# chzchzchz/raftsql

Measured on NVIDIA B200. Metric: raft_ticks_per_sec_1Mx5, higher is better.
Workload: dtype u64

## Files before the change

raftsql_b200/csrc/mrq_kernels.cuh:

```cuda
#pragma once

#include <cuda_runtime.h>
#include <stdint.h>

#include "../../include/mrq.h"
#include "../../include/mrq_packed8.h"
#include "../../include/mrq_trace.h"

namespace mrq {

static constexpr uint64_t kNoGate = 0xFFFFFFFFFFFFFFFFull;

struct Meta {
  uint32_t role, lead, vote, self, elapsed, rto, hb, votes, strict, ltok;
};
__host__ __device__ __forceinline__ uint64_t meta_pack(const Meta &m) {
  return (uint64_t)(m.role & 3u) | ((uint64_t)(m.lead & 15u) << 2) | ((uint64_t)(m.vote & 15u) << 6) |
         ((uint64_t)(m.self & 15u) << 10) | ((uint64_t)(m.elapsed & 0xFFFu) << 14) |
         ((uint64_t)(m.rto & 0xFFFu) << 26) | ((uint64_t)(m.hb & 0xFFu) << 38) |
         ((uint64_t)(m.votes & 0xFFFFu) << 46) | ((uint64_t)(m.strict & 1u) << 62) | ((uint64_t)(m.ltok & 1u) << 63);
}
__host__ __device__ __forceinline__ Meta meta_unpack(uint64_t w) {
  Meta m;
  m.role = (uint32_t)(w & 3u);
// ... 31 lines not shown
  uint64_t *tick_next;
  uint32_t election_tick, heartbeat_tick;
  uint8_t *peer_lo[8];
  uint64_t *peer_full[8];
  uint32_t world, rank, gather_prime;
  uint32_t l2_policy;
  uint32_t *slow_list;
  unsigned *slow_count, *slow_count_next;
};

__device__ __forceinline__ void pdl_launch_dependents() { asm volatile("griddepcontrol.launch_dependents;"); }
__device__ __forceinline__ void pdl_wait() { asm volatile("griddepcontrol.wait;" ::: "memory"); }

template <class Args>
__device__ __forceinline__ void gather_store(const Args &a, const uint64_t i, const uint64_t committed, const uint64_t committed0) {
  const uint64_t at = (uint64_t)a.rank * a.G + i;
  const bool full = a.gather_prime || ((committed ^ committed0) >> 8) != 0;
#pragma unroll 1
  for (uint32_t p = 0; p < a.world; ++p) {
    a.peer_lo[p][at] = (uint8_t)committed;
    if (full) a.peer_full[p][at] = committed;
  }
}

#ifndef MRQ_HOST_EMULATION
__device__ __forceinline__ uint64_t ld_stream(const uint64_t *p) {
  uint64_t v;
  asm volatile("ld.global.nc.L1::no_allocate.u64 %0, [%1];" : "=l"(v) : "l"(p));
  return v;
}
__device__ __forceinline__ uint32_t ld_stream_u8(const uint8_t *p) {
  uint32_t v;
  asm volatile("ld.global.nc.L1::no_allocate.u8 %0, [%1];" : "=r"(v) : "l"(p));
  return v;
}
__device__ __forceinline__ uint32_t ld_stream_u32(const uint32_t *p) {
  uint32_t v;
  asm volatile("ld.global.nc.L1::no_allocate.u32 %0, [%1];" : "=r"(v) : "l"(p));
  return v;
}
__device__ __forceinline__ uint64_t ld_state(const uint64_t *p) {
  uint64_t v;
  asm volatile("ld.global.L1::no_allocate.u64 %0, [%1];" : "=l"(v) : "l"(p));
  return v;
}
__device__ __forceinline__ void st_state(uint64_t *p, uint64_t v) {
  asm volatile("st.global.L1::no_allocate.u64 [%0], %1;" ::"l"(p), "l"(v) : "memory");
}
__device__ __forceinline__ void st_state_u32(uint32_t *p, uint32_t v) {
  asm volatile("st.global.L1::no_allocate.u32 [%0], %1;" ::"l"(p), "r"(v) : "memory");
}

__device__ __forceinline__ uint64_t l2_policy(uint32_t kind) {
  uint64_t p;
  if (kind == 1u)
    asm volatile("createpolicy.fractional.L2::evict_first.b64 %0, 1.0;" : "=l"(p));
  else if (kind == 2u)
    asm volatile("createpolicy.fractional.L2::evict_last.b64 %0, 1.0;" : "=l"(p));
  else
    asm volatile("createpolicy.fractional.L2::evict_normal.b64 %0, 1.0;" : "=l"(p));
  return p;
}
__device__ __forceinline__ uint64_t ld_stream_p(const uint64_t *p, uint64_t pol) {
  uint64_t v;
  asm volatile("ld.global.nc.L1::no_allocate.L2::cache_hint.u64 %0, [%1], %2;" : "=l"(v) : "l"(p), "l"(pol));
  return v;
}
__device__ __forceinline__ uint32_t ld_stream_u8_p(const uint8_t *p, uint64_t pol) {
  uint32_t v;
  asm volatile("ld.global.nc.L1::no_allocate.L2::cache_hint.u8 %0, [%1], %2;" : "=r"(v) : "l"(p), "l"(pol));
  return v;
}
__device__ __forceinline__ uint32_t ld_stream_u32_p(const uint32_t *p, uint64_t pol) {
  uint32_t v;
  asm volatile("ld.global.nc.L1::no_allocate.L2::cache_hint.u32 %0, [%1], %2;" : "=r"(v) : "l"(p), "l"(pol));
  return v;
}
__device__ __forceinline__ uint64_t ld_state_p(const uint64_t *p, uint64_t pol) {
  uint64_t v;
  asm volatile("ld.global.L1::no_allocate.L2::cache_hint.u64 %0, [%1], %2;" : "=l"(v) : "l"(p), "l"(pol));
  return v;
}
__device__ __forceinline__ void st_state_p(uint64_t *p, uint64_t v, uint64_t pol) {
  asm volatile("st.global.L1::no_allocate.L2::cache_hint.u64 [%0], %1, %2;" ::"l"(p), "l"(v), "l"(pol) : "memory");
}
__device__ __forceinline__ void st_state_u32_p(uint32_t *p, uint32_t v, uint64_t pol) {
  asm volatile("st.global.L1::no_allocate.L2::cache_hint.u32 [%0], %1, %2;" ::"l"(p), "r"(v), "l"(pol) : "memory");
}
#else
inline uint64_t ld_stream(const uint64_t *p) { return *p; }
inline uint32_t ld_stream_u8(const uint8_t *p) { return *p; }
inline uint32_t ld_stream_u32(const uint32_t *p) { return *p; }
inline uint64_t ld_state(const uint64_t *p) { return *p; }
inline void st_state(uint64_t *p, uint64_t v) { *p = v; }
inline void st_state_u32(uint32_t *p, uint32_t v) { *p = v; }
inline uint64_t l2_policy(uint32_t) { return 0; }
inline uint64_t ld_stream_p(const uint64_t *p, uint64_t) { return *p; }
inline uint32_t ld_stream_u8_p(const uint8_t *p, uint64_t) { return *p; }
inline uint32_t ld_stream_u32_p(const uint32_t *p, uint64_t) { return *p; }
inline uint64_t ld_state_p(const uint64_t *p, uint64_t) { return *p; }
inline void st_state_p(uint64_t *p, uint64_t v, uint64_t) { *p = v; }
inline void st_state_u32_p(uint32_t *p, uint32_t v, uint64_t) { *p = v; }
#endif

__device__ __forceinline__ void cswap_desc(uint64_t &hi, uint64_t &lo) {
  const uint64_t a = hi, b = lo;
  const bool sw = a < b;
  hi = sw ? b : a;
  lo = sw ? a : b;
}
template <int R>
__device__ __forceinline__ uint64_t quorum_index64(const uint64_t (&m)[R]) {
  constexpr int Q = R / 2 + 1;
  uint64_t v[R];
#pragma unroll
  for (int i = 0; i < R; ++i) v[i] = m[i];
#pragma unroll
  for (int p = 0; p < Q; ++p) {
#pragma unroll
    for (int i = R - 1; i > p; --i) cswap_desc(v[i - 1], v[i]);
  }
  return v[Q - 1];
}
template <int R>
__device__ __forceinline__ uint32_t quorum_index32(const uint32_t (&d)[R]) {
  constexpr int Q = R / 2 + 1;
  if constexpr (R == 1) {
    return d[0];
  } else if constexpr (R == 2) {
    return min(d[0], d[1]);
  } else if constexpr (R == 3) {
    return max(min(d[0], d[1]), min(max(d[0], d[1]), d[2]));
  } else if constexpr (R == 5) {
    const uint32_t lo_ab = min(d[0], d[1]), hi_ab = max(d[0], d[1]);
    const uint32_t lo_cd = min(d[2], d[3]), hi_cd = max(d[2], d[3]);
    const uint32_t f = max(lo_ab, lo_cd), g = min(hi_ab, hi_cd);
    return max(min(d[4], f), min(max(d[4], f), g));
  } else {
    uint32_t v[R];
#pragma unroll
    for (int i = 0; i < R; ++i) v[i] = d[i];
#pragma unroll
    for (int p = 0; p < Q; ++p) {
#pragma unroll
      for (int i = R - 1; i > p; --i) {
        const uint32_t a = v[i - 1], b = v[i];
        v[i - 1] = max(a, b);
        v[i] = min(a, b);
      }
    }
    return v[Q - 1];
  }
}
__device__ __forceinline__ void delta32(uint64_t m, uint64_t c, uint32_t &d, uint32_t &bad) {
  uint32_t lo, hi, b;
#ifndef MRQ_HOST_EMULATION
  asm("sub.cc.u32 %0, %3, %5;\n\t"
      "subc.cc.u32 %1, %4, %6;\n\t"
      "subc.u32 %2, 0, 0;"
      : "=r"(lo), "=r"(hi), "=r"(b)
      : "r"((uint32_t)m), "r"((uint32_t)(m >> 32)), "r"((uint32_t)c), "r"((uint32_t)(c >> 32)));
#else
  const uint64_t diff = m - c;
  lo = (uint32_t)diff;
  hi = (uint32_t)(diff >> 32);
  b = m < c ? 0xFFFFFFFFu : 0u;
#endif
  d = ((b | hi) == 0u) ? lo : 0u;
  bad |= ~b & hi;
}
template <int R>
__device__ __forceinline__ uint64_t quorum_index(const uint64_t (&m)[R], uint64_t committed) {
  uint32_t d[R];
  uint32_t bad = 0;
#pragma unroll
  for (int r = 0; r < R; ++r) delta32(m[r], committed, d[r], bad);
  if (__builtin_expect(bad == 0u, 1)) return committed + quorum_index32<R>(d);
  return quorum_index64<R>(m);
}

enum : uint32_t {
  D_TERM = 1u << 0, D_LI = 1u << 1, D_LT = 1u << 2, D_COMMIT = 1u << 3, D_GATE = 1u << 4, D_MATCH0 = 1u << 8
};

template <int R>
struct Group {
  uint64_t term, last_index, last_term, committed, gate;
  uint64_t match[R];
  uint32_t role, lead, vote, self, elapsed, rto, hb, votes, strict, ltok;
  uint32_t out, dirty, ev;
  bool lt_valid;
  bool pending;
  const uint64_t *lt_ptr;
  uint64_t seed, gg, tick_no;
  uint32_t et, ht;

  static constexpr uint32_t Q = R / 2 + 1;
  enum : uint32_t { EV_CAMPAIGN = 1, EV_WON = 2, EV_STEPDOWN = 4, EV_COMMIT = 8, EV_GRANT = 16, EV_ERROR = 32 };

  __device__ __forceinline__ uint64_t lastTerm() {
    if (!lt_valid) {
      last_term = ltok ? term : ld_state(lt_ptr);
      lt_valid = true;
    }
    return last_term;
  }
  __device__ __forceinline__ void setSelfMatch(uint64_t v) {
#pragma unroll
    for (int r = 0; r < R; ++r)
      if ((uint32_t)(r + 1) == self && match[r] != v) {
        match[r] = v;
        dirty |= D_MATCH0 << r;
      }
  }
  __device__ __forceinline__ bool maybeCommit() {
    const uint64_t mci = quorum_index<R>(match, committed);
    if (mci > committed && mci >= gate && mci <= last_index) {
      committed = mci;
      dirty |= D_COMMIT;
      out |= MRQ_OUT_COMMIT_ADVANCED;
      ev |= EV_COMMIT;
      return true;
    }
    return false;
  }
  __device__ __forceinline__ void flushCommit() {
    if (pending) {
      pending = false;
      if (maybeCommit()) out |= MRQ_OUT_BCAST_APPEND;
    }
  }
  __device__ __forceinline__ void reset(uint64_t t) {
    if (term != t) {
      term = t;
      vote = 0;
      ltok = 0;
      dirty |= D_TERM;
    }
    lead = 0;
    elapsed = 0;
    hb = 0;
    votes = 0;
    rto = mrq_randomized_timeout(seed, gg, tick_no, et);
  }
  __device__ __forceinline__ void becomeFollower(uint64_t t, uint32_t ld) {
    flushCommit();
    if (role != MRQ_ROLE_FOLLOWER) {
      out |= MRQ_OUT_STEPPED_DOWN;
      ev |= EV_STEPDOWN;
    }
    reset(t);
    lead = ld;
    role = MRQ_ROLE_FOLLOWER;
    if (gate != kNoGate) {
      gate = kNoGate;
      dirty |= D_GATE;
    }
  }
  __device__ __forceinline__ void appendEntry(uint32_t n) {
    last_index += n;
    dirty |= D_LI;
    if (!ltok && (!lt_valid || last_term != term)) {
      last_term = term;
      lt_valid = true;
      dirty |= D_LT;
    }
    ltok = 1;
    setSelfMatch(last_index);
    pending = false;
    maybeCommit();
  }
  __device__ __forceinline__ void becomeLeader() {
    reset(term);
    lead = self;
    role = MRQ_ROLE_LEADER;
    strict = 0;
    pending = false;
    out |= MRQ_OUT_BECAME_LEADER;
    ev |= EV_WON;
#pragma unroll
    for (int r = 0; r < R; ++r) {
      match[r] = 0;
      dirty |= D_MATCH0 << r;
    }
    gate = last_index + 1;
    dirty |= D_GATE;
    appendEntry(1);
  }
  __device__ __forceinline__ void campaign() {
    reset(term + 1);
    vote = self;
    role = MRQ_ROLE_CANDIDATE;
    ev |= EV_CAMPAIGN;
    votes |= 1u << (2u * (self - 1u));
    if (Q == 1u) {
      becomeLeader();
      return;
    }
    out |= MRQ_OUT_CAMPAIGN;
  }
  __device__ __forceinline__ void commitTo(uint64_t c) {
    if (committed < c) {
      if (last_index < c) {
        ev |= EV_ERROR;
        return;
      }
// ... 571 lines not shown
  for (unsigned it = 0; it < rounds; ++it, k += stride) {
    uint32_t ev = 0;
    if (k < n) ev = general_group_tick<R>(a, (uint64_t)a.slow_list[k]);
    if (__any_sync(0xFFFFFFFFu, ev != 0)) count_events(a.ctr, ev);
  }
}

struct Tick8Args {
  TickArgs t;
  Inbox8 b;
};
template <int R>
__global__ void __launch_bounds__(kTickThreads, (R <= 5 ? 8 : (R == 6 ? 7 : 6))) tick_fast8_kernel(const Tick8Args a8) {
  const TickArgs &a = a8.t;
  pdl_launch_dependents();
  const uint64_t i = (uint64_t)blockIdx.x * blockDim.x + threadIdx.x;
  uint32_t ev = 0;
  bool slow = false;
  pdl_wait();
  if (blockIdx.x == 0 && threadIdx.x == 0) *a.tick_next = *a.tick_cur + 1;
  fast_group_tick8<R>(a, a8.b, i, slow, ev);
  const unsigned smask = __ballot_sync(0xFFFFFFFFu, slow);
  if (smask != 0) {
    const unsigned lane = threadIdx.x & 31u;
    unsigned base = 0;
    if (lane == 0) base = atomicAdd(a.slow_count, (unsigned)__popc(smask));
    base = __shfl_sync(0xFFFFFFFFu, base, 0);
    if (slow) a.slow_list[base + __popc(smask & ((1u << lane) - 1u))] = (uint32_t)i;
  }
  if (__any_sync(0xFFFFFFFFu, ev != 0)) count_events(a.ctr, ev);
}
template <int R>
__global__ void __launch_bounds__(kTickThreads, (R <= 5 ? 6 : 5)) tick_slow8_kernel(const Tick8Args a8) {
  const TickArgs &a = a8.t;
  pdl_launch_dependents();
  pdl_wait();
  const unsigned n = *a.slow_count;
  if (blockIdx.x == 0 && threadIdx.x == 0) *a.slow_count_next = 0;
  const unsigned stride = gridDim.x * blockDim.x;
  const unsigned rounds = (n + stride - 1) / stride;
  unsigned k = blockIdx.x * blockDim.x + threadIdx.x;
  for (unsigned it = 0; it < rounds; ++it, k += stride) {
    uint32_t ev = 0;
    if (k < n) ev = general_group_tick8<R>(a, a8.b, (uint64_t)a.slow_list[k]);
    if (__any_sync(0xFFFFFFFFu, ev != 0)) count_events(a.ctr, ev);
  }
}

template <int R>
__global__ void __launch_bounds__(kTickThreads, (R <= 5 ? 6 : 5)) tick_fused_kernel(const TickArgs a) {
  __shared__ uint32_t s_list[kTickThreads];
  __shared__ unsigned s_n;
  pdl_launch_dependents();
  const uint64_t base = (uint64_t)blockIdx.x * blockDim.x;
  uint32_t ev = 0;
  bool slow = false;
  if (threadIdx.x == 0) s_n = 0;
  pdl_wait();
  if (blockIdx.x == 0 && threadIdx.x == 0) *a.tick_next = *a.tick_cur + 1;
  fast_group_tick<R>(a, base + threadIdx.x, slow, ev);
  __syncthreads();
  const unsigned smask = __ballot_sync(0xFFFFFFFFu, slow);
  if (smask != 0) {
    const unsigned lane = threadIdx.x & 31u;
    unsigned pos = 0;
    if (lane == 0) pos = atomicAdd(&s_n, (unsigned)__popc(smask));
    pos = __shfl_sync(0xFFFFFFFFu, pos, 0);
    if (slow) s_list[pos + __popc(smask & ((1u << lane) - 1u))] = threadIdx.x;
  }
  __syncthreads();
  const unsigned n = s_n;
  if (__any_sync(0xFFFFFFFFu, ev != 0)) count_events(a.ctr, ev);
  if (n != 0) {
    uint32_t ev2 = 0;
    if (threadIdx.x < n) ev2 = general_group_tick<R>(a, base + s_list[threadIdx.x]);
    if (__any_sync(0xFFFFFFFFu, ev2 != 0)) count_events(a.ctr, ev2);
  }
}

template <int R>
__global__ void __launch_bounds__(kTickThreads, (R <= 5 ? 6 : 5)) tick_general_kernel(const TickArgs a) {
  pdl_launch_dependents();
  const uint64_t i = (uint64_t)blockIdx.x * blockDim.x + threadIdx.x;
  pdl_wait();
  if (blockIdx.x == 0 && threadIdx.x == 0) *a.tick_next = *a.tick_cur + 1;
  uint32_t ev = 0;
  if (i < a.G) ev = general_group_tick<R>(a, i);
  if (__any_sync(0xFFFFFFFFu, ev != 0)) count_events(a.ctr, ev);
}

enum : uint32_t { CF_COMPACT = 1u, CF_TERM_OK = 2u, CF_GATE_OPEN = 4u };
enum : uint32_t { CD_META = 1u, CD_COMMIT = 2u, CD_WIN = 4u, CD_MATCH0 = 1u << 8, CD_MATCH_ANY = 0xFFu << 8 };
#ifndef MRQ_HOST_EMULATION
static constexpr uint32_t kCompactSpan = 0x7FFFFFFFu;
#else
static uint32_t kCompactSpan = 0x7FFFFFFFu;
#endif

struct CompactView {
  uint8_t *flag;
  uint32_t *commit;
  uint32_t *win;
  uint32_t *gate;
  uint32_t *iblo;
  uint32_t *match;
  uint64_t *ibase;
};

template <int R>
struct CGroup {
  uint64_t meta;
  uint32_t commit, win;
  uint32_t m[R];
};

__host__ __device__ __forceinline__ uint32_t crow_sender(uint32_t j, uint32_t self_id) {
  return j + (j + 1u >= self_id ? 1u : 0u);
}

template <int R>
__device__ __forceinline__ bool compact_hot_step(CGroup<R> &g, const uint32_t flag, const uint32_t (&wb)[R > 1 ? R - 1 : 1],
                                                 const uint32_t nprop, const uint32_t gate, const uint32_t et, const uint32_t ht,
                                                 uint32_t &out, uint32_t &adv, uint32_t &dirty) {
  constexpr uint64_t kSettled = 3ull | (1ull << 62) | (1ull << 63);
  bool hot = (flag & (CF_COMPACT | CF_TERM_OK)) == (CF_COMPACT | CF_TERM_OK) &&
             (g.meta & kSettled) == ((uint64_t)MRQ_ROLE_LEADER | (1ull << 63));
  uint32_t li = g.m[R - 1];
  hot = hot && li + nprop <= kCompactSpan;
  uint32_t nm[R];
  uint32_t d = 0, min_ack = MRQ_P8_NO_ACK, kinds = 0, mx_max = 0, moved = 0;
#pragma unroll
  for (int j = 0; j < R - 1; ++j) {
    const uint32_t w = wb[j];
    kinds |= w;
    const bool ack = (w & 1u) != 0u;
    const uint32_t pay = w >> 2;
    const uint32_t mx = ack ? g.win + pay : 0u;
    mx_max = max(mx_max, mx);
    nm[j] = max(g.m[j], mx);
    moved |= nm[j] ^ g.m[j];
    min_ack = ack ? min(min_ack, pay) : min_ack;
  }
  if (!hot || mx_max > li || (kinds & 2u) != 0u) return false;
  uint32_t o = 0;
  li += nprop;
  nm[R - 1] = li;
  if (nprop) {
    moved = 1u;
    o |= MRQ_OUT_BCAST_APPEND;
  }
  d = moved != 0u ? CD_MATCH0 : 0u;
  uint32_t commit = g.commit, q = 0;
  if (d != 0u) {
    uint32_t dl[R];
#pragma unroll
    for (int r = 0; r < R; ++r) dl[r] = max(nm[r], commit) - commit;
    q = quorum_index32<R>(dl);
    const bool open = (flag & CF_GATE_OPEN) != 0u || commit + q >= gate;
    q = (commit + q <= li && open) ? q : 0u;
  }
  if (q != 0u) {
    commit += q;
    d |= CD_COMMIT;
    o |= MRQ_OUT_COMMIT_ADVANCED | MRQ_OUT_BCAST_APPEND;
  }
  uint32_t lo = (uint32_t)g.meta, hi = (uint32_t)(g.meta >> 32);
  uint32_t el = ((lo >> 14) & 0xFFFu) + 1u;
  el = el >= et ? 0u : el;
  lo = (lo & ~(0xFFFu << 14)) | (el << 14);
  if (ht <= 1u) {
    hi &= ~(0xFFu << 6);
    o |= MRQ_OUT_BCAST_HEARTBEAT;
  } else {
    uint32_t hb = ((hi >> 6) & 0xFFu) + 1u;
    if (hb >= ht) {
      hb = 0;
      o |= MRQ_OUT_BCAST_HEARTBEAT;
    }
    hi = (hi & ~(0xFFu << 6)) | (hb << 6);
  }
  const uint64_t nmeta = ((uint64_t)hi << 32) | lo;
  d |= nmeta != g.meta ? CD_META : 0u;
  if (min_ack < MRQ_P8_NO_ACK && min_ack > MRQ_P8_SLACK) {
    g.win += min_ack - MRQ_P8_SLACK;
    d |= CD_WIN;
  }
  g.meta = nmeta;
  g.commit = commit;
#pragma unroll
  for (int r = 0; r < R; ++r) g.m[r] = nm[r];
  out = o;
  adv = q;
  dirty = d;
  return true;
}

template <int R>
__device__ __forceinline__ bool compact_step(CGroup<R> &g, const uint32_t flag, const uint32_t (&wb)[R > 1 ? R - 1 : 1],
                                             const uint32_t nprop, const uint32_t gate, const uint32_t et, const uint32_t ht,
                                             uint32_t &out, uint32_t &adv, uint32_t &dirty) {
  out = 0;
  adv = 0;
  dirty = 0;
  if (!(flag & CF_COMPACT)) return true;
  Meta m = meta_unpack(g.meta);
  uint32_t kind[R > 1 ? R - 1 : 1], pay[R > 1 ? R - 1 : 1];
  bool any_ack = false, any_hb = false;
  uint32_t min_ack = MRQ_P8_NO_ACK;
#pragma unroll
  for (int j = 0; j < R - 1; ++j) {
    kind[j] = wb[j] & 3u;
    pay[j] = (wb[j] >> 2) & 63u;
    if (kind[j] == 1u) {
      any_ack = true;
      min_ack = pay[j] < min_ack ? pay[j] : min_ack;
    } else if (kind[j] == 3u) {
      any_hb = true;
    } else if (kind[j] == 2u && (pay[j] <= 2u || pay[j] == 63u)) {
      return true;
    } else {
      kind[j] = 0;
    }
  }
  uint32_t li = g.m[R - 1];
  CGroup<R> n = g;
  if (m.role == MRQ_ROLE_LEADER) {
    if (m.strict || !m.ltok || any_hb) return true;
    if (any_ack && !(flag & CF_TERM_OK)) return true;
    if (li + nprop > kCompactSpan) return true;
    bool changed = false;
#pragma unroll
    for (int j = 0; j < R - 1; ++j)
      if (kind[j] == 1u) {
        const uint32_t mx = g.win + pay[j];
        if (mx > li) return true;
        if (n.m[j] < mx) {
          n.m[j] = mx;
          dirty |= CD_MATCH0 << j;
          changed = true;
        }
      }
    if (nprop) {
      li += nprop;
      n.m[R - 1] = li;
      dirty |= CD_MATCH0 << (R - 1);
      out |= MRQ_OUT_BCAST_APPEND;
      changed = true;
    }
    if (changed) {
      uint32_t d[R];
#pragma unroll
      for (int r = 0; r < R; ++r) d[r] = max(n.m[r], n.commit) - n.commit;
      const uint32_t q = quorum_index32<R>(d);
      const uint32_t mci = n.commit + q;
      if (q != 0u && mci <= li && ((flag & CF_GATE_OPEN) != 0u || mci >= gate)) {
        adv = q;
        n.commit = mci;
        dirty |= CD_COMMIT;
        out |= MRQ_OUT_COMMIT_ADVANCED | MRQ_OUT_BCAST_APPEND;
      }
    }
    ++m.hb;
    ++m.elapsed;
    if (m.elapsed >= et) m.elapsed = 0;
    if (m.hb >= ht) {
      m.hb = 0;
      out |= MRQ_OUT_BCAST_HEARTBEAT;
    }
  } else if (m.role == MRQ_ROLE_FOLLOWER) {
    if (nprop != 0u || any_ack) return true;
    if (any_hb && !(flag & CF_TERM_OK)) return true;
#pragma unroll
    for (int j = 0; j < R - 1; ++j)
      if (kind[j] == 3u && (crow_sender((uint32_t)j, m.self) + 1u != m.lead || g.win + pay[j] > li)) return true;
    if ((any_hb ? 1u : m.elapsed + 1u) >= m.rto) return true;
#pragma unroll
    for (int j = 0; j < R - 1; ++j)
      if (kind[j] == 3u) {
        const uint32_t mx = g.win + pay[j];
        if (n.commit < mx) {
          adv += mx - n.commit;
          n.commit = mx;
          dirty |= CD_COMMIT;
          out |= MRQ_OUT_COMMIT_ADVANCED;
        }
        out |= 1u << (MRQ_OUT_ACK_REPLY_SHIFT + crow_sender((uint32_t)j, m.self));
      }
    m.elapsed = any_hb ? 1u : m.elapsed + 1u;
  } else {
    return true;
  }
  if (min_ack < MRQ_P8_NO_ACK && min_ack > MRQ_P8_SLACK) {
    n.win = g.win + (min_ack - MRQ_P8_SLACK);
    dirty |= CD_WIN;
  }
  n.meta = meta_pack(m);
  if (n.meta != g.meta) dirty |= CD_META;
  g = n;
  return false;
}

__device__ __forceinline__ void materialise_group(const StateView &s, const CompactView &c, uint64_t *base_index, uint64_t gs, uint32_t R,
                                                  const uint64_t i) {
  if (!(c.flag[i] & CF_COMPACT)) return;
  const Meta m = meta_unpack(s.meta[i]);
  const uint64_t ib = c.ibase[i];
  s.committed[i] = ib + c.commit[i];
  base_index[i] = ib + c.win[i];
  s.last_index[i] = ib + c.match[(uint64_t)(R - 1u) * gs + i];
  if (m.role == MRQ_ROLE_LEADER) {
    s.match[(uint64_t)(m.self - 1u) * gs + i] = ib + c.match[(uint64_t)(R - 1u) * gs + i];
    for (uint32_t j = 0; j + 1u < R; ++j) {
      const uint32_t v = c.match[(uint64_t)j * gs + i];
      if (v != 0u) s.match[(uint64_t)crow_sender(j, m.self) * gs + i] = ib + v;
    }
  }
}

__device__ __forceinline__ void compact_group(const StateView &s, const CompactView &c, const uint64_t *base_index,
                                              const uint64_t *base_term, uint64_t gs, uint32_t R, const uint64_t i) {
  const Meta m = meta_unpack(s.meta[i]);
  const uint64_t li = s.last_index[i], cm = s.committed[i], wb = base_index[i], gate = s.term_start[i];
  const uint64_t lo = cm < wb ? cm : wb;
  const uint64_t ib = lo ? lo - 1u : 0u;
  bool fits = m.self >= 1 && m.self <= R && !m.strict && cm <= li && li - ib <= (uint64_t)kCompactSpan &&
              wb - ib <= (uint64_t)kCompactSpan;
  const bool leader = m.role == MRQ_ROLE_LEADER;
  if (fits && leader) fits = s.match[(uint64_t)(m.self - 1u) * gs + i] == li;
  if (!fits) {
    c.flag[i] = 0;
    return;
  }
  c.ibase[i] = ib;
  c.iblo[i] = (uint32_t)ib;
  c.commit[i] = (uint32_t)(cm - ib);
  c.win[i] = (uint32_t)(wb - ib);
  for (uint32_t j = 0; j + 1u < R; ++j) {
    uint32_t v = 0;
    if (leader) {
      const uint64_t mv = s.match[(uint64_t)crow_sender(j, m.self) * gs + i];
      v = mv > ib ? (uint32_t)(mv - ib) : 0u;
    }
    c.match[(uint64_t)j * gs + i] = v;
  }
  c.match[(uint64_t)(R - 1u) * gs + i] = (uint32_t)(li - ib);
  uint32_t go = 0xFFFFFFFFu;
  if (leader) go = gate > ib ? (gate - ib > 0xFFFFFFFEull ? 0xFFFFFFFFu : (uint32_t)(gate - ib)) : 0u;
  c.gate[i] = go;
  c.flag[i] = (uint8_t)(CF_COMPACT | (base_term[i] == s.term[i] ? CF_TERM_OK : 0u) | ((leader && gate <= cm) ? CF_GATE_OPEN : 0u));
}

struct TickDesc {
  const uint8_t *word8;
  const uint8_t *prop8;
  InboxView in;
  uint32_t *out;
  uint8_t *delta;
};
static constexpr uint32_t kMaxTicksPerLaunch = 96;
struct Tick4Args {
  TickArgs t;
  CompactView c;
  uint64_t *base_index;
  const uint64_t *base_term;
  TickDesc d0;
  const TickDesc *descs;
  uint32_t nticks;
  uint32_t write_through;
  unsigned long long *slow_list64;
};

template <int R>
__device__ __forceinline__ uint32_t slow_group_ticks_c(const Tick4Args &A, const uint64_t i, const uint32_t t0) {
  const TickArgs &a0 = A.t;
  materialise_group(a0.s, A.c, A.base_index, a0.gs, (uint32_t)R, i);
  uint32_t ev = 0;
  const uint64_t tick0 = *a0.tick_cur;
  for (uint32_t t = t0; t < A.nticks; ++t) {
    const TickDesc d = A.descs ? A.descs[t] : A.d0;
    TickArgs a = a0;
    a.in = d.in;
    a.s.out = d.out;
    const uint64_t c0 = a.s.committed[i];
    const Inbox8 b{d.word8, d.prop8, A.base_index, A.base_term};
    ev |= general_group_tick8<R>(a, b, i, tick0 + t);
    const uint64_t adv = a.s.committed[i] - c0;
    d.delta[i] = (uint8_t)(adv > 255u ? 255u : adv);
  }
  compact_group(a0.s, A.c, A.base_index, A.base_term, a0.gs, (uint32_t)R, i);
  return ev;
}

#ifndef MRQ_HOST_EMULATION
template <int R>
struct CStepResult {
  CGroup<R> g;
  uint32_t out, adv, dirty, slow;
};
template <int R>
__device__ __noinline__ CStepResult<R> compact_step_cold(CGroup<R> g, uint32_t flag, uint32_t w0123, uint32_t w4567, uint32_t nprop,
                                                         uint32_t gate, uint32_t et, uint32_t ht) {
  uint32_t wb[R > 1 ? R - 1 : 1];
#pragma unroll
  for (int j = 0; j < (R > 1 ? R - 1 : 1); ++j) wb[j] = ((j < 4 ? w0123 : w4567) >> (8 * (j & 3))) & 0xFFu;
  CStepResult<R> r;
  r.slow = compact_step<R>(g, flag, wb, nprop, gate, et, ht, r.out, r.adv, r.dirty) ? 1u : 0u;
  r.g = g;
  return r;
}
#endif

#ifndef MRQ_HOST_EMULATION
struct u32x4 {
  uint32_t v[4];
};
__device__ __forceinline__ u32x4 ld_v4u32_p(const uint32_t *p, uint64_t pol) {
  u32x4 r;
  asm volatile("ld.global.L1::no_allocate.L2::cache_hint.v4.u32 {%0, %1, %2, %3}, [%4], %5;"
               : "=r"(r.v[0]), "=r"(r.v[1]), "=r"(r.v[2]), "=r"(r.v[3])
               : "l"(p), "l"(pol));
  return r;
}
__device__ __forceinline__ void st_v4u32_p(uint32_t *p, const u32x4 &r, uint64_t pol) {
  asm volatile("st.global.L1::no_allocate.L2::cache_hint.v4.u32 [%0], {%1, %2, %3, %4}, %5;" ::"l"(p), "r"(r.v[0]), "r"(r.v[1]),
               "r"(r.v[2]), "r"(r.v[3]), "l"(pol)
               : "memory");
}
__device__ __forceinline__ void ld_v2u64_p(const uint64_t *p, uint64_t pol, uint64_t &a, uint64_t &b) {
  asm volatile("ld.global.L1::no_allocate.L2::cache_hint.v2.u64 {%0, %1}, [%2], %3;" : "=l"(a), "=l"(b) : "l"(p), "l"(pol));
}
__device__ __forceinline__ void st_v2u64_p(uint64_t *p, uint64_t a, uint64_t b, uint64_t pol) {
  asm volatile("st.global.L1::no_allocate.L2::cache_hint.v2.u64 [%0], {%1, %2}, %3;" ::"l"(p), "l"(a), "l"(b), "l"(pol) : "memory");
}

template <int R, int THREADS>
#ifndef MRQ_T4_THREADS_PER_SM
#define MRQ_T4_THREADS_PER_SM 512
#endif
__global__ void __launch_bounds__(THREADS, (R <= 5 ? MRQ_T4_THREADS_PER_SM : 384) / THREADS) tick_fast4_kernel(const Tick4Args A) {
  const TickArgs &a = A.t;
  pdl_launch_dependents();
  const uint64_t i0 = ((uint64_t)blockIdx.x * blockDim.x + threadIdx.x) * 4u;
  const bool active = i0 < a.gs;
  const uint64_t i = active ? i0 : 0;
  const uint64_t pol_stream = l2_policy(a.l2_policy ? 1u : 0u);
  const uint64_t pol_keep = l2_policy(a.l2_policy ? 2u : 0u);
  pdl_wait();
  if (blockIdx.x == 0 && threadIdx.x == 0) *a.tick_next = *a.tick_cur + A.nticks;
  CGroup<R> g[4];
  uint32_t flag[4];
  {
    const uint32_t fw = ld_stream_u32_p(reinterpret_cast<const uint32_t *>(A.c.flag + i), pol_keep);
    ld_v2u64_p(a.s.meta + i, pol_keep, g[0].meta, g[1].meta);
    ld_v2u64_p(a.s.meta + i + 2, pol_keep, g[2].meta, g[3].meta);
    const u32x4 cm = ld_v4u32_p(A.c.commit + i, pol_keep);
    const u32x4 wn = ld_v4u32_p(A.c.win + i, pol_keep);
    u32x4 mv[R];
#pragma unroll
    for (int r = 0; r < R; ++r) mv[r] = ld_v4u32_p(A.c.match + (uint64_t)r * a.gs + i, pol_keep);
#pragma unroll
    for (int k = 0; k < 4; ++k) {
      flag[k] = (fw >> (8 * k)) & 0xFFu;
      g[k].commit = cm.v[k];
      g[k].win = wn.v[k];
#pragma unroll
      for (int r = 0; r < R; ++r) g[k].m[r] = mv[r].v[k];
    }
  }
  uint32_t stopped = 0;
#pragma unroll
  for (int k = 0; k < 4; ++k)
    if (!active || i0 + k >= a.G) stopped |= 1u << k;
  u32x4 gate{};
  if (((flag[0] & flag[1] & flag[2] & flag[3]) & CF_GATE_OPEN) == 0u) gate = ld_v4u32_p(A.c.gate + i, pol_keep);
  const bool gather = a.world > 1;
  u32x4 iblo{};
  if (gather) iblo = ld_v4u32_p(A.c.iblo + i, pol_keep);
  uint32_t acc_dirty = 0, ncommit = 0;
  __shared__ TickDesc s_desc[kMaxTicksPerLaunch];
  if (A.descs) {
    const uint32_t nw = A.nticks * (uint32_t)(sizeof(TickDesc) / 4);
    for (uint32_t w = threadIdx.x; w < nw; w += THREADS) reinterpret_cast<uint32_t *>(s_desc)[w] = reinterpret_cast<const uint32_t *>(A.descs)[w];
  } else if (threadIdx.x == 0) {
    s_desc[0] = A.d0;
  }
  __syncthreads();
  constexpr int NW = R > 1 ? R - 1 : 1;
  auto load_frame = [&](uint32_t t, uint32_t (&w)[NW], uint32_t &pbytes) {
    const TickDesc &dd = s_desc[t];
#pragma unroll
    for (int j = 0; j < R - 1; ++j) w[j] = ld_stream_u32_p(reinterpret_cast<const uint32_t *>(dd.word8 + (uint64_t)j * a.gs + i), pol_stream);
    if (R == 1) w[0] = 0;
    pbytes = dd.prop8 ? ld_stream_u32_p(reinterpret_cast<const uint32_t *>(dd.prop8 + i), pol_stream) : 0u;
  };
  uint32_t wb[NW], pb, wb1[NW], pb1 = 0;
  load_frame(0, wb, pb);
#pragma unroll
  for (int j = 0; j < NW; ++j) wb1[j] = 0;
  if (A.nticks > 1) load_frame(1, wb1, pb1);
  for (uint32_t t = 0; t < A.nticks; ++t) {
    uint32_t wb2[NW], pb2 = 0;
#pragma unroll
    for (int j = 0; j < NW; ++j) wb2[j] = 0;
    if (t + 2 < A.nticks) load_frame(t + 2, wb2, pb2);
    const TickDesc &d = s_desc[t];
    u32x4 outw{};
    uint32_t dw = 0, newly = 0, tdirty = 0;
    u32x4 lo_old{};
    if (gather) {
#pragma unroll
      for (int k = 0; k < 4; ++k) lo_old.v[k] = iblo.v[k] + g[k].commit;
    }
#pragma unroll
    for (int k = 0; k < 4; ++k) {
      if (stopped & (1u << k)) continue;
      uint32_t wk[R > 1 ? R - 1 : 1];
#pragma unroll
      for (int j = 0; j < (R > 1 ? R - 1 : 1); ++j) wk[j] = (wb[j] >> (8 * k)) & 0xFFu;
      uint32_t o, adv, dirty;
      const uint32_t np = (pb >> (8 * k)) & 0xFFu;
      bool slow = false;
      if (!compact_hot_step<R>(g[k], flag[k], wk, np, gate.v[k], a.election_tick, a.heartbeat_tick, o, adv, dirty)) {
        uint32_t p0 = 0, p1 = 0;
#pragma unroll
        for (int j = 0; j < R - 1; ++j) {
          if (j < 4) p0 |= wk[j] << (8 * j);
          else p1 |= wk[j] << (8 * (j - 4));
        }
        const CStepResult<R> cr = compact_step_cold<R>(g[k], flag[k], p0, p1, np, gate.v[k], a.election_tick, a.heartbeat_tick);
        g[k] = cr.g;
        o = cr.out;
        adv = cr.adv;
        dirty = cr.dirty;
        slow = cr.slow != 0u;
      }
      if (slow) {
        newly |= 1u << k;
      } else {
        outw.v[k] = o;
        dw |= (adv > 255u ? 255u : adv) << (8 * k);
        tdirty |= dirty;
        ncommit += adv != 0u;
      }
    }
    if (__any_sync(0xFFFFFFFFu, newly != 0u)) {
#pragma unroll
      for (int k = 0; k < 4; ++k) {
        const bool s = (newly >> k) & 1u;
        const unsigned smask = __ballot_sync(0xFFFFFFFFu, s);
        if (smask != 0) {
          const unsigned lane = threadIdx.x & 31u;
          unsigned base = 0;
          if (lane == 0) base = atomicAdd(a.slow_count, (unsigned)__popc(smask));
          base = __shfl_sync(0xFFFFFFFFu, base, 0);
          if (s) A.slow_list64[base + __popc(smask & ((1u << lane) - 1u))] = ((unsigned long long)t << 32) | (unsigned long long)(i0 + k);
        }
      }
      stopped |= newly;
    }
    acc_dirty |= tdirty;
    if (active) {
      st_v4u32_p(d.out + i, outw, pol_stream);
      st_state_u32_p(reinterpret_cast<uint32_t *>(d.delta + i), dw, pol_stream);
      if (gather) {
        uint32_t lo4 = 0;
        bool carry = false;
        u32x4 lo;
#pragma unroll
        for (int k = 0; k < 4; ++k) {
          lo.v[k] = iblo.v[k] + g[k].commit;
          lo4 |= (lo.v[k] & 0xFFu) << (8 * k);
          carry = carry || ((lo.v[k] ^ lo_old.v[k]) >> 8) != 0u;
        }
        const uint64_t at = (uint64_t)a.rank * a.G + i;
        const bool whole = i0 + 3 < a.G && (at & 3u) == 0u && stopped == 0u;
#pragma unroll 1
        for (uint32_t p = 0; p < a.world; ++p) {
          if (whole) {
            st_state_u32_p(reinterpret_cast<uint32_t *>(a.peer_lo[p] + at), lo4, pol_stream);
          } else {
#pragma unroll
            for (int k = 0; k < 4; ++k)
              if (!(stopped & (1u << k))) a.peer_lo[p][at + k] = (uint8_t)lo.v[k];
          }
        }
        if (a.gather_prime || carry) {
#pragma unroll
          for (int k = 0; k < 4; ++k)
            if (!(stopped & (1u << k)) && (a.gather_prime || ((lo.v[k] ^ lo_old.v[k]) >> 8) != 0u)) {
              const uint64_t full = A.c.ibase[i + k] + g[k].commit;
#pragma unroll 1
              for (uint32_t p = 0; p < a.world; ++p) a.peer_full[p][at + k] = full;
            }
        }
      }
    }
    const bool last = t + 1 == A.nticks;
    if (A.write_through || last) {
      uint32_t wd = __reduce_or_sync(0xFFFFFFFFu, A.write_through ? tdirty : acc_dirty);
      if (active) {
        if (wd & CD_META) {
          st_v2u64_p(a.s.meta + i, g[0].meta, g[1].meta, pol_keep);
          st_v2u64_p(a.s.meta + i + 2, g[2].meta, g[3].meta, pol_keep);
        }
        if (wd & CD_COMMIT) st_v4u32_p(A.c.commit + i, u32x4{{g[0].commit, g[1].commit, g[2].commit, g[3].commit}}, pol_keep);
        if (wd & CD_WIN) st_v4u32_p(A.c.win + i, u32x4{{g[0].win, g[1].win, g[2].win, g[3].win}}, pol_keep);
        if (wd & CD_MATCH_ANY) {
#pragma unroll
          for (int r = 0; r < R; ++r)
            st_v4u32_p(A.c.match + (uint64_t)r * a.gs + i, u32x4{{g[0].m[r], g[1].m[r], g[2].m[r], g[3].m[r]}}, pol_keep);
        }
      }
    }
#pragma unroll
    for (int j = 0; j < NW; ++j) {
      wb[j] = wb1[j];
      wb1[j] = wb2[j];
    }
    pb = pb1;
    pb1 = pb2;
  }
  const unsigned tot = __reduce_add_sync(0xFFFFFFFFu, ncommit);
  if (tot != 0 && (threadIdx.x & 31u) == 0)
    atomicAdd(&a.ctr[blockIdx.x & (kCtrShards - 1)].commits_advanced, (unsigned long long)tot);
}

template <int R>
__global__ void __launch_bounds__(128, 7) tick_fast1_kernel(const Tick4Args A) {
  const TickArgs &a = A.t;
  pdl_launch_dependents();
  const uint64_t i0 = (uint64_t)blockIdx.x * blockDim.x + threadIdx.x;
  const bool valid = i0 < a.G;
  const uint64_t i = i0 < a.gs ? i0 : 0;
  const uint64_t pol_stream = l2_policy(a.l2_policy ? 1u : 0u);
  const uint64_t pol_keep = l2_policy(a.l2_policy ? 2u : 0u);
  pdl_wait();
  if (blockIdx.x == 0 && threadIdx.x == 0) *a.tick_next = *a.tick_cur + A.nticks;
  __shared__ TickDesc s_desc[kMaxTicksPerLaunch];
  if (A.descs) {
    const uint32_t nw = A.nticks * (uint32_t)(sizeof(TickDesc) / 4);
    for (uint32_t w = threadIdx.x; w < nw; w += blockDim.x) reinterpret_cast<uint32_t *>(s_desc)[w] = reinterpret_cast<const uint32_t *>(A.descs)[w];
  } else if (threadIdx.x == 0) {
    s_desc[0] = A.d0;
  }
  __syncthreads();
  CGroup<R> g;
  const uint32_t flag = ld_stream_u8_p(A.c.flag + i, pol_keep);
  g.meta = ld_state_p(a.s.meta + i, pol_keep);
  g.commit = ld_stream_u32_p(A.c.commit + i, pol_keep);
  g.win = ld_stream_u32_p(A.c.win + i, pol_keep);
#pragma unroll
  for (int r = 0; r < R; ++r) g.m[r] = ld_stream_u32_p(A.c.match + (uint64_t)r * a.gs + i, pol_keep);
  const uint32_t gate = (flag & CF_GATE_OPEN) ? 0u : ld_stream_u32_p(A.c.gate + i, pol_keep);
  const bool gather = a.world > 1;
  const uint32_t iblo = gather ? ld_stream_u32_p(A.c.iblo + i, pol_keep) : 0u;
  constexpr int NW = R > 1 ? R - 1 : 1;
  auto load_frame = [&](uint32_t t, uint32_t (&w)[NW], uint32_t &np) {
    const TickDesc &dd = s_desc[t];
#pragma unroll
    for (int j = 0; j < R - 1; ++j) w[j] = ld_stream_u8_p(dd.word8 + (uint64_t)j * a.gs + i, pol_stream);
    if (R == 1) w[0] = 0;
    np = dd.prop8 ? ld_stream_u8_p(dd.prop8 + i, pol_stream) : 0u;
  };
  uint32_t wb[NW], pb, wb1[NW], pb1 = 0;
  load_frame(0, wb, pb);
#pragma unroll
  for (int j = 0; j < NW; ++j) wb1[j] = 0;
  if (A.nticks > 1) load_frame(1, wb1, pb1);
  bool stopped = !valid;
  uint32_t acc_dirty = 0, ncommit = 0;
  __shared__ __align__(16) uint8_t s_lo[128];
  const bool cta_gather = gather && (uint64_t)(blockIdx.x + 1u) * 128u <= a.G && (((uint64_t)a.rank * a.G) & 3u) == 0u;
  for (uint32_t t = 0; t < A.nticks; ++t) {
    uint32_t wb2[NW], pb2 = 0;
#pragma unroll
    for (int j = 0; j < NW; ++j) wb2[j] = 0;
    if (t + 2 < A.nticks) load_frame(t + 2, wb2, pb2);
    const TickDesc &d = s_desc[t];
    uint32_t o = 0, adv = 0, dirty = 0;
    bool newly = false;
    const uint32_t lo_old = iblo + g.commit;
    if (!stopped) {
      if (!compact_hot_step<R>(g, flag, wb, pb, gate, a.election_tick, a.heartbeat_tick, o, adv, dirty)) {
        uint32_t p0 = 0, p1 = 0;
#pragma unroll
        for (int j = 0; j < R - 1; ++j) {
          if (j < 4) p0 |= wb[j] << (8 * j);
          else p1 |= wb[j] << (8 * (j - 4));
        }
        const CStepResult<R> cr = compact_step_cold<R>(g, flag, p0, p1, pb, gate, a.election_tick, a.heartbeat_tick);
        g = cr.g;
        o = cr.out;
        adv = cr.adv;
        dirty = cr.dirty;
        newly = cr.slow != 0u;
      }
      if (newly) {
        o = 0;
        adv = 0;
        dirty = 0;
      }
      ncommit += adv != 0u;
    }
    const unsigned smask = __ballot_sync(0xFFFFFFFFu, newly);
    if (smask != 0) {
      const unsigned lane = threadIdx.x & 31u;
      unsigned base = 0;
      if (lane == 0) base = atomicAdd(a.slow_count, (unsigned)__popc(smask));
      base = __shfl_sync(0xFFFFFFFFu, base, 0);
      if (newly) A.slow_list64[base + __popc(smask & ((1u << lane) - 1u))] = ((unsigned long long)t << 32) | (unsigned long long)i0;
      stopped = stopped || newly;
    }
    acc_dirty |= dirty;
    if (valid) {
      st_state_u32_p(d.out + i, o, pol_stream);
      d.delta[i] = (uint8_t)(adv > 255u ? 255u : adv);
      if (gather && !cta_gather && !stopped) {
        const uint32_t lo = iblo + g.commit;
        const uint64_t at = (uint64_t)a.rank * a.G + i;
#pragma unroll 1
        for (uint32_t p = 0; p < a.world; ++p) a.peer_lo[p][at] = (uint8_t)lo;
      }
      if (gather && !stopped) {
        const uint32_t lo = iblo + g.commit;
        if (a.gather_prime || ((lo ^ lo_old) >> 8) != 0u) {
          const uint64_t at = (uint64_t)a.rank * a.G + i;
          const uint64_t fv = A.c.ibase[i] + g.commit;
#pragma unroll 1
          for (uint32_t p = 0; p < a.world; ++p) a.peer_full[p][at] = fv;
        }
      }
    }
    if (cta_gather) {
      s_lo[threadIdx.x] = (uint8_t)(iblo + g.commit);
      __syncthreads();
      const uint32_t word = reinterpret_cast<const uint32_t *>(s_lo)[threadIdx.x & 31u];
      const uint64_t at0 = (uint64_t)a.rank * a.G + (uint64_t)blockIdx.x * 128u;
      for (uint32_t p = threadIdx.x >> 5; p < a.world; p += 4u)
        st_state_u32_p(reinterpret_cast<uint32_t *>(a.peer_lo[p] + at0) + (threadIdx.x & 31u), word, pol_stream);
      __syncthreads();
    }
    const bool last = t + 1 == A.nticks;
    if (A.write_through || last) {
      const uint32_t wd = __reduce_or_sync(0xFFFFFFFFu, A.write_through ? dirty : acc_dirty);
      if (valid) {
        if (wd & CD_META) st_state_p(a.s.meta + i, g.meta, pol_keep);
        if (wd & CD_COMMIT) st_state_u32_p(A.c.commit + i, g.commit, pol_keep);
        if (wd & CD_WIN) st_state_u32_p(A.c.win + i, g.win, pol_keep);
        if (wd & CD_MATCH_ANY) {
#pragma unroll
          for (int r = 0; r < R; ++r) st_state_u32_p(A.c.match + (uint64_t)r * a.gs + i, g.m[r], pol_keep);
        }
      }
    }
#pragma unroll
    for (int j = 0; j < NW; ++j) {
      wb[j] = wb1[j];
      wb1[j] = wb2[j];
    }
    pb = pb1;
    pb1 = pb2;
  }
  const unsigned tot = __reduce_add_sync(0xFFFFFFFFu, ncommit);
  if (tot != 0 && (threadIdx.x & 31u) == 0)
    atomicAdd(&a.ctr[blockIdx.x & (kCtrShards - 1)].commits_advanced, (unsigned long long)tot);
}

template <int R>
__global__ void __launch_bounds__(kTickThreads, (R <= 5 ? 6 : 5)) tick_slow4_kernel(const Tick4Args A) {
  const TickArgs &a = A.t;
  pdl_launch_dependents();
  pdl_wait();
  const unsigned n = *a.slow_count;
// ... 517 lines not shown
```

Baseline: 109,200.

## Add SIMD-within-register quad hot path and self-max quorum selection for compact ticks

Adds a fast path that steps all four groups a thread owns together while they are settled leaders. It packs per-byte ack minimum and maximum with SWAR byte compares and applies timer updates through precomputed thresholds. Quorum selection now takes the median over the raw match values of the peers and then clamps against commit, which removes the per-element subtraction. The frame ring is rotated by unrolling the tick loop three ways instead of copying registers. Non-eligible quads fall back to a noinline per-group step, which adds register pressure and code size and risks subtle semantic differences in the new fast path.

```diff
diff --git a/raftsql_b200/csrc/mrq_kernels.cuh b/raftsql_b200/csrc/mrq_kernels.cuh
--- a/raftsql_b200/csrc/mrq_kernels.cuh
+++ b/raftsql_b200/csrc/mrq_kernels.cuh
@@ -207,6 +207,29 @@
     return v[Q - 1];
   }
 }
+template <int R>
+__device__ __forceinline__ uint32_t quorum_index_selfmax(const uint32_t (&m)[R]) {
+  constexpr int K = R / 2;
+  if constexpr (K == 0) {
+    return m[R - 1];
+  } else if constexpr (R == 5) {
+    return max(min(max(m[0], m[1]), max(m[2], m[3])), max(min(m[0], m[1]), min(m[2], m[3])));
+  } else {
+    uint32_t v[R - 1];
+#pragma unroll
+    for (int i = 0; i < R - 1; ++i) v[i] = m[i];
+#pragma unroll
+    for (int p = 0; p < K; ++p) {
+#pragma unroll
+      for (int i = R - 2; i > p; --i) {
+        const uint32_t a = v[i - 1], b = v[i];
+        v[i - 1] = max(a, b);
+        v[i] = min(a, b);
+      }
+    }
+    return v[K - 1];
+  }
+}
 __device__ __forceinline__ void delta32(uint64_t m, uint64_t c, uint32_t &d, uint32_t &bad) {
   uint32_t lo, hi, b;
 #ifndef MRQ_HOST_EMULATION
@@ -1084,10 +1107,7 @@
   d = moved != 0u ? CD_MATCH0 : 0u;
   uint32_t commit = g.commit, q = 0;
   if (d != 0u) {
-    uint32_t dl[R];
-#pragma unroll
-    for (int r = 0; r < R; ++r) dl[r] = max(nm[r], commit) - commit;
-    q = quorum_index32<R>(dl);
+    q = max(quorum_index_selfmax<R>(nm), commit) - commit;
     const bool open = (flag & CF_GATE_OPEN) != 0u || commit + q >= gate;
     q = (commit + q <= li && open) ? q : 0u;
   }
@@ -1230,6 +1250,107 @@
   if (n.meta != g.meta) dirty |= CD_META;
   g = n;
   return false;
+}
+
+__device__ __forceinline__ uint32_t quad_byte(uint32_t w, int k) {
+#ifndef MRQ_HOST_EMULATION
+  return __byte_perm(w, 0u, 0x4440u + (uint32_t)k);
+#else
+  return (w >> (8 * k)) & 0xFFu;
+#endif
+}
+__device__ __forceinline__ uint32_t bytes_ge7(uint32_t a, uint32_t b) {
+  return (((a | 0x80808080u) - b) >> 7 & 0x01010101u) * 0xFFu;
+}
+
+template <int R>
+__device__ __forceinline__ bool quad_hot_eligible(const CGroup<R> (&g)[4], const uint32_t (&flag)[4], uint32_t stopped) {
+  constexpr uint64_t kSettled = 3ull | (1ull << 62) | (1ull << 63);
+  bool ok = stopped == 0u;
+#pragma unroll
+  for (int k = 0; k < 4; ++k)
+    ok = ok && (flag[k] & (CF_COMPACT | CF_TERM_OK)) == (CF_COMPACT | CF_TERM_OK) &&
+         (g[k].meta & kSettled) == ((uint64_t)MRQ_ROLE_LEADER | (1ull << 63));
+  return ok;
+}
+
+struct HotTimers {
+  uint32_t el_reset;
+  uint32_t hb_reset;
+  uint32_t hb_beat;
+};
+__device__ __forceinline__ HotTimers hot_timers(uint32_t et, uint32_t ht) {
+  const uint32_t e1 = et ? et - 1u : 0u, h1 = ht ? ht - 1u : 0u;
+  return HotTimers{min(e1, 0xFFFu) << 14, min(h1, 0xFFu) << 6, min(h1, 0x100u) << 6};
+}
+
+template <int R>
+__device__ __forceinline__ bool compact_hot_quad(CGroup<R> (&g)[4], const uint32_t (&w)[R > 1 ? R - 1 : 1], const uint32_t pw,
+                                                 const uint32_t (&gate)[4], const HotTimers &tm, uint32_t (&out)[4], uint32_t &dw,
+                                                 uint32_t &dirty, uint32_t &nadv) {
+  constexpr uint32_t kEl = 0xFFFu << 14, kHb = 0xFFu << 6;
+  uint32_t kinds = 0, emin = MRQ_P8_NO_ACK * 0x01010101u, amax = 0;
+  uint32_t e[R > 1 ? R - 1 : 1];
+#pragma unroll
+  for (int j = 0; j < R - 1; ++j) {
+    kinds |= w[j];
+    const uint32_t ack = w[j] & 0x01010101u;
+    const uint32_t a = (w[j] >> 2) & (ack * 0x3Fu);
+    e[j] = a | (0x40404040u - (ack << 6));
+    const uint32_t lt = bytes_ge7(emin, e[j]);
+    emin = (emin & ~lt) | (e[j] & lt);
+    const uint32_t ge = bytes_ge7(amax, a);
+    amax = (amax & ge) | (a & ~ge);
+  }
+  if ((kinds & 0x02020202u) != 0u) return false;
+  bool bad = false;
+#pragma unroll
+  for (int k = 0; k < 4; ++k) {
+    const uint32_t li = g[k].m[R - 1];
+    bad = bad || quad_byte(pw, k) + li > kCompactSpan || (quad_byte(emin, k) < MRQ_P8_NO_ACK && g[k].win + quad_byte(amax, k) > li);
+  }
+  if (bad) return false;
+  uint32_t d = CD_META, adv4 = 0, n = 0;
+#pragma unroll
+  for (int k = 0; k < 4; ++k) {
+    CGroup<R> &G = g[k];
+    const uint32_t np = quad_byte(pw, k);
+    uint32_t nm[R], moved = np;
+#pragma unroll
+    for (int j = 0; j < R - 1; ++j) {
+      const uint32_t ek = quad_byte(e[j], k);
+      nm[j] = ek < MRQ_P8_NO_ACK ? max(G.m[j], G.win + ek) : G.m[j];
+      moved |= nm[j] ^ G.m[j];
+    }
+    const uint32_t li = G.m[R - 1] + np;
+    nm[R - 1] = li;
+    const uint32_t mci = max(quorum_index_selfmax<R>(nm), G.commit);
+    const uint32_t q = (moved != 0u && mci <= li && mci >= gate[k]) ? mci - G.commit : 0u;
+    uint32_t o = (np | q) != 0u ? MRQ_OUT_BCAST_APPEND : 0u;
+    o |= q != 0u ? MRQ_OUT_COMMIT_ADVANCED : 0u;
+    d |= (moved != 0u ? CD_MATCH0 : 0u) | (q != 0u ? CD_COMMIT : 0u);
+    G.commit += q;
+    adv4 |= min(q, 255u) << (8 * k);
+    n += q != 0u;
+    uint32_t lo = (uint32_t)G.meta, hi = (uint32_t)(G.meta >> 32);
+    const uint32_t el = lo & kEl, hb = hi & kHb;
+    lo = el >= tm.el_reset ? lo - el : lo + (1u << 14);
+    hi = hb >= tm.hb_reset ? hi - hb : hi + (1u << 6);
+    o |= hb >= tm.hb_beat ? MRQ_OUT_BCAST_HEARTBEAT : 0u;
+    G.meta = ((uint64_t)hi << 32) | lo;
+    const uint32_t mn = quad_byte(emin, k);
+    if (mn - (MRQ_P8_SLACK + 1u) < MRQ_P8_NO_ACK - (MRQ_P8_SLACK + 1u)) {
+      G.win += mn - MRQ_P8_SLACK;
+      d |= CD_WIN;
+    }
+#pragma unroll
+    for (int r = 0; r < R; ++r) G.m[r] = nm[r];
+    out[k] = o;
+  }
+  dw = adv4;
+  dirty = d;
+  nadv = n;
+  return true;
 }
 
 __device__ __forceinline__ void materialise_group(const StateView &s, const CompactView &c, uint64_t *base_index, uint64_t gs, uint32_t R,
@@ -1338,6 +1459,50 @@
   CStepResult<R> r;
   r.slow = compact_step<R>(g, flag, wb, nprop, gate, et, ht, r.out, r.adv, r.dirty) ? 1u : 0u;
   r.g = g;
+  return r;
+}
+
+template <int R>
+struct QuadFrame {
+  uint32_t w[R > 1 ? R - 1 : 1];
+  uint32_t p;
+};
+template <int R>
+struct QuadState {
+  CGroup<R> g[4];
+};
+template <int R>
+struct QuadStep {
+  CGroup<R> g[4];
+  uint32_t out[4], dw, dirty, newly, nadv;
+};
+template <int R>
+__device__ __noinline__ QuadStep<R> quad_step_each(const QuadState<R> s, const uint32_t fw, const QuadFrame<R> f, const uint4 gate,
+                                                   const uint32_t stopped, const uint32_t et, const uint32_t ht) {
+  QuadStep<R> r;
+  r.dw = r.dirty = r.newly = r.nadv = 0;
+  const uint32_t gv[4] = {gate.x, gate.y, gate.z, gate.w};
+#pragma unroll
+  for (int k = 0; k < 4; ++k) {
+    r.g[k] = s.g[k];
+    r.out[k] = 0;
+    if (stopped & (1u << k)) continue;
+    const uint32_t flag = (fw >> (8 * k)) & 0xFFu, np = (f.p >> (8 * k)) & 0xFFu;
+    uint32_t wk[R > 1 ? R - 1 : 1] = {0};
+#pragma unroll
+    for (int j = 0; j < R - 1; ++j) wk[j] = (f.w[j] >> (8 * k)) & 0xFFu;
+    uint32_t o, adv, dirty;
+    if (!compact_hot_step<R>(r.g[k], flag, wk, np, gv[k], et, ht, o, adv, dirty)) {
+      if (compact_step<R>(r.g[k], flag, wk, np, gv[k], et, ht, o, adv, dirty)) {
+        r.newly |= 1u << k;
+        continue;
+      }
+    }
+    r.out[k] = o;
+    r.dw |= (adv > 255u ? 255u : adv) << (8 * k);
+    r.dirty |= dirty;
+    r.nadv += adv != 0u;
+  }
   return r;
 }
 #endif
@@ -1417,64 +1582,49 @@
     s_desc[0] = A.d0;
   }
   __syncthreads();
-  constexpr int NW = R > 1 ? R - 1 : 1;
-  auto load_frame = [&](uint32_t t, uint32_t (&w)[NW], uint32_t &pbytes) {
+  auto load_frame = [&](uint32_t t, QuadFrame<R> &f) {
     const TickDesc &dd = s_desc[t];
 #pragma unroll
-    for (int j = 0; j < R - 1; ++j) w[j] = ld_stream_u32_p(reinterpret_cast<const uint32_t *>(dd.word8 + (uint64_t)j * a.gs + i), pol_stream);
-    if (R == 1) w[0] = 0;
-    pbytes = dd.prop8 ? ld_stream_u32_p(reinterpret_cast<const uint32_t *>(dd.prop8 + i), pol_stream) : 0u;
+    for (int j = 0; j < R - 1; ++j) f.w[j] = ld_stream_u32_p(reinterpret_cast<const uint32_t *>(dd.word8 + (uint64_t)j * a.gs + i), pol_stream);
+    if (R == 1) f.w[0] = 0;
+    f.p = dd.prop8 ? ld_stream_u32_p(reinterpret_cast<const uint32_t *>(dd.prop8 + i), pol_stream) : 0u;
   };
-  uint32_t wb[NW], pb, wb1[NW], pb1 = 0;
-  load_frame(0, wb, pb);
-#pragma unroll
-  for (int j = 0; j < NW; ++j) wb1[j] = 0;
-  if (A.nticks > 1) load_frame(1, wb1, pb1);
-  for (uint32_t t = 0; t < A.nticks; ++t) {
-    uint32_t wb2[NW], pb2 = 0;
-#pragma unroll
-    for (int j = 0; j < NW; ++j) wb2[j] = 0;
-    if (t + 2 < A.nticks) load_frame(t + 2, wb2, pb2);
+  const HotTimers tm = hot_timers(a.election_tick, a.heartbeat_tick);
+  uint32_t fw = 0, hgate[4];
+#pragma unroll
+  for (int k = 0; k < 4; ++k) {
+    fw |= flag[k] << (8 * k);
+    hgate[k] = (flag[k] & CF_GATE_OPEN) ? 0u : gate.v[k];
+  }
+  bool hot = quad_hot_eligible<R>(g, flag, stopped);
+  auto tick = [&](const uint32_t t, const QuadFrame<R> &f, QuadFrame<R> &ahead) {
+    if (t + 2 < A.nticks) load_frame(t + 2, ahead);
     const TickDesc &d = s_desc[t];
     u32x4 outw{};
-    uint32_t dw = 0, newly = 0, tdirty = 0;
+    uint32_t dw = 0, newly = 0, tdirty = 0, nadv = 0;
     u32x4 lo_old{};
     if (gather) {
 #pragma unroll
       for (int k = 0; k < 4; ++k) lo_old.v[k] = iblo.v[k] + g[k].commit;
     }
-#pragma unroll
-    for (int k = 0; k < 4; ++k) {
-      if (stopped & (1u << k)) continue;
-      uint32_t wk[R > 1 ? R - 1 : 1];
-#pragma unroll
-      for (int j = 0; j < (R > 1 ? R - 1 : 1); ++j) wk[j] = (wb[j] >> (8 * k)) & 0xFFu;
-      uint32_t o, adv, dirty;
-      const uint32_t np = (pb >> (8 * k)) & 0xFFu;
-      bool slow = false;
-      if (!compact_hot_step<R>(g[k], flag[k], wk, np, gate.v[k], a.election_tick, a.heartbeat_tick, o, adv, dirty)) {
-        uint32_t p0 = 0, p1 = 0;
-#pragma unroll
-        for (int j = 0; j < R - 1; ++j) {
-          if (j < 4) p0 |= wk[j] << (8 * j);
-          else p1 |= wk[j] << (8 * (j - 4));
-        }
-        const CStepResult<R> cr = compact_step_cold<R>(g[k], flag[k], p0, p1, np, gate.v[k], a.election_tick, a.heartbeat_tick);
-        g[k] = cr.g;
-        o = cr.out;
-        adv = cr.adv;
-        dirty = cr.dirty;
-        slow = cr.slow != 0u;
-      }
-      if (slow) {
-        newly |= 1u << k;
-      } else {
-        outw.v[k] = o;
-        dw |= (adv > 255u ? 255u : adv) << (8 * k);
-        tdirty |= dirty;
-        ncommit += adv != 0u;
-      }
-    }
+    if (!(hot && compact_hot_quad<R>(g, f.w, f.p, hgate, tm, outw.v, dw, tdirty, nadv))) {
+      QuadState<R> qs;
+#pragma unroll
+      for (int k = 0; k < 4; ++k) qs.g[k] = g[k];
+      const QuadStep<R> r = quad_step_each<R>(qs, fw, f, make_uint4(gate.v[0], gate.v[1], gate.v[2], gate.v[3]), stopped,
+                                              a.election_tick, a.heartbeat_tick);
+#pragma unroll
+      for (int k = 0; k < 4; ++k) {
+        g[k] = r.g[k];
+        outw.v[k] = r.out[k];
+      }
+      dw = r.dw;
+      tdirty = r.dirty;
+      newly = r.newly;
+      nadv = r.nadv;
+      hot = quad_hot_eligible<R>(g, flag, stopped | newly);
+    }
+    ncommit += nadv;
     if (__any_sync(0xFFFFFFFFu, newly != 0u)) {
 #pragma unroll
       for (int k = 0; k < 4; ++k) {
@@ -1544,13 +1694,16 @@
         }
       }
     }
-#pragma unroll
-    for (int j = 0; j < NW; ++j) {
-      wb[j] = wb1[j];
-      wb1[j] = wb2[j];
-    }
-    pb = pb1;
-    pb1 = pb2;
+  };
+  QuadFrame<R> fa, fb{}, fc{};
+  load_frame(0, fa);
+  if (A.nticks > 1) load_frame(1, fb);
+  for (uint32_t t = 0; t < A.nticks; t += 3) {
+    tick(t, fa, fc);
+    if (t + 1 >= A.nticks) break;
+    tick(t + 1, fb, fa);
+    if (t + 2 >= A.nticks) break;
+    tick(t + 2, fc, fb);
   }
   const unsigned tot = __reduce_add_sync(0xFFFFFFFFu, ncommit);
   if (tot != 0 && (threadIdx.x & 31u) == 0)
```

After: 111,900 (median of 6 runs). 1.03x the previous value.
